# zertovitch/zip-ada

Measured on AMD Instinct MI355X. Metric: Deflate encode MB/s (Deflate_3; stream bit-exact with the CPU restatement of the reference, Ada parity unpinned), higher is better.
Workload: dtype u8

## Files before the change

### zip-ada_amd/csrc/zada_api.hip

```cpp
#include <hip/hip_runtime.h>
#include <stdint.h>
#include <stdio.h>
#include <string.h>
#include <algorithm>
#include <new>
#include <atomic>
#include <mutex>
#include <condition_variable>
#include <functional>
#include <thread>
#include "../../include/zada.h"
#include "zada_internal.h"
#include "zada_bt4.h"

struct zada_ctx { zada::Ctx c; };

namespace zada {

thread_local std::string *tls_err = nullptr;
int hip_check(Ctx *c, hipError_t e, const char *what) {
  if (e == hipSuccess) return 0;
  char buf[256];
  snprintf(buf, sizeof buf, "%s: %s", what, hipGetErrorString(e));
  if (tls_err) *tls_err = buf; else c->err = buf;
// ... 890 lines not shown
  lzma_free(&z->c);
  free_workspace(&z->c);
  for (hipEvent_t e : z->c.ev_pool) hipEventDestroy(e);
  if (z->c.stream2) hipStreamDestroy(z->c.stream2);
  if (z->c.crc_host) hipHostFree(z->c.crc_host);
  for (int b = 0; b < 2 * MAX_COPY_LANES; b++) { if (z->c.stage[b]) hipHostFree(z->c.stage[b]); if (z->c.ev_stage[b]) hipEventDestroy(z->c.ev_stage[b]); }
  for (int t = 0; t < MAX_COPY_LANES; t++) { if (z->c.stream_in[t]) hipStreamDestroy(z->c.stream_in[t]); if (z->c.ev_in[t]) hipEventDestroy(z->c.ev_in[t]); }
  if (z->c.bstage) hipHostFree(z->c.bstage);
  if (z->c.btab) hipHostFree(z->c.btab);
  if (z->c.ev_input) hipEventDestroy(z->c.ev_input);
  if (z->c.ev_out) hipEventDestroy(z->c.ev_out);
  if (z->c.ev_dlim) hipEventDestroy(z->c.ev_dlim);
  if (z->c.stream) hipStreamDestroy(z->c.stream);
  delete z;
}

zada_ctx *zada_create(int device) {
  int ndev = 0;
  if (hipGetDeviceCount(&ndev) != hipSuccess || ndev <= 0 || device < 0 || device >= ndev) return nullptr;
  if (hipSetDevice(device) != hipSuccess) return nullptr;
  zada_ctx *z = new (std::nothrow) zada_ctx();
  if (!z) return nullptr;
  z->c.device = device;
  if (hipStreamCreate(&z->c.stream) != hipSuccess ||
      hipHostMalloc((void **)&z->c.crc_host, (CRC_HOST_TOP + 64) * 4, hipHostMallocDefault) != hipSuccess ||
      hipStreamCreate(&z->c.stream2) != hipSuccess || hipEventCreateWithFlags(&z->c.ev_input, hipEventDisableTiming) != hipSuccess ||
      hipEventCreateWithFlags(&z->c.ev_out, hipEventDisableTiming) != hipSuccess || hipEventCreateWithFlags(&z->c.ev_dlim, hipEventDisableTiming) != hipSuccess) { (void)hipGetLastError(); ctx_release(z); return nullptr; }
  if (const char *e = getenv("ZADA_BUDGET")) z->c.knob_budget = atoi(e);
  if (const char *e = getenv("ZADA_INNER_BUDGET")) z->c.knob_inner_budget = atoi(e);
  if (const char *e = getenv("ZADA_LINK_RUN")) { const int v = atoi(e); if (v >= 0 && v <= 64 && !(v & (v - 1))) z->c.knob_link_run = v; }
  if (const char *e = getenv("ZADA_ATOMS_PCT")) { if (atoi(e) >= 1 && atoi(e) <= 100) z->c.knob_atoms_pct = atoi(e); }
  if (const char *e = getenv("ZADA_CD_FILTER")) z->c.knob_cd_filter = atoi(e) != 0;
  if (const char *e = getenv("ZADA_EXACT_RESPEC")) { if (atoi(e) >= 0) z->c.knob_exact_respec = atoi(e); }
  if (const char *e = getenv("ZADA_MAX_DEMAND_ROUNDS")) { if (atoi(e) > 0) z->c.knob_max_demand_rounds = atoi(e); }
  if (const char *e = getenv("ZADA_SHARD_KIB")) { if (atoi(e) >= 64 && atoi(e) % 64 == 0) z->c.knob_shard_kib = atoi(e); }
  return z;
}

void zada_destroy(zada_ctx *z) {
  if (!z) return;
  hipSetDevice(z->c.device);
  ctx_release(z);
}

const char *zada_last_error(const zada_ctx *z) { return z ? z->c.err.c_str() : "no context"; }

int zada_set_knob(zada_ctx *z, const char *name, int value) {
  if (!z || !name) return ZADA_E_INVALID;
  if (!strcmp(name, "budget")) z->c.knob_budget = value;
  else if (!strcmp(name, "inner_budget")) z->c.knob_inner_budget = value;
  else if (!strcmp(name, "link_run")) { if (value < 0 || value > 64 || (value & (value - 1))) return ZADA_E_INVALID; z->c.knob_link_run = value; }
  else if (!strcmp(name, "span_mib")) { if (value < 1 || value > 3968) return ZADA_E_INVALID; z->c.knob_span_mib = value; }
  else if (!strcmp(name, "bunzip_batch_mib")) { if (value < 16 || value > 262144) return ZADA_E_INVALID; z->c.knob_bunzip_batch_mib = value; }
  else if (!strcmp(name, "bz_batch_mib")) { if (value < 1 || value > 2048) return ZADA_E_INVALID; z->c.knob_bz_batch_mib = value; }
  else if (!strcmp(name, "bz_span_mib")) { if (value < 24 || value > 3072) return ZADA_E_INVALID; z->c.knob_bz_span_mib = value; }
  else if (!strcmp(name, "bz_batch_melems")) { if (value < 1 || value > 1536) return ZADA_E_INVALID; z->c.knob_bz_batch_melems = value; }
  else if (!strcmp(name, "bz_tail_pct")) { if (value < 0 || value > 50) return ZADA_E_INVALID; z->c.knob_bz_tail_pct = value; }
  else if (!strcmp(name, "bz_text_order")) { if (value < 0 || value > 1) return ZADA_E_INVALID; z->c.knob_bz_text_order = value; }
  else if (!strcmp(name, "bz_pipeline")) { if (value < 0 || value > 1) return ZADA_E_INVALID; z->c.knob_bz_pipeline = value; }
  else if (!strcmp(name, "bz_pipe_prio")) { if (value < 0 || value > 1) return ZADA_E_INVALID; z->c.knob_bz_pipe_prio = value; }
  else if (!strcmp(name, "bz_list_rows")) { if (value < 0 || value > 8192) return ZADA_E_INVALID; z->c.knob_bz_list_rows = value; }
  else if (!strcmp(name, "bz_split")) { if (value < 0 || value > 1) return ZADA_E_INVALID; z->c.knob_bz_split = value; }
  else if (!strcmp(name, "bz_small_wg")) { if (value < 0 || value > 1) return ZADA_E_INVALID; z->c.knob_bz_small_wg = value; }
  else if (!strcmp(name, "bz_lists")) { if (value < -1) return ZADA_E_INVALID; z->c.knob_bz_lists = value; }
  else if (!strcmp(name, "batch_mib")) { if (value < 1 || value > 1024) return ZADA_E_INVALID; z->c.knob_batch_mib = value; }
  else if (!strcmp(name, "atoms_pct")) { if (value < 1 || value > 100) return ZADA_E_INVALID; z->c.knob_atoms_pct = value; z->c.ws.cap_atoms = 0; }
  else if (!strcmp(name, "fix_stride")) { if (value < 0 || value > (int)PTOK_STRIDE) return ZADA_E_INVALID; z->c.knob_fix_stride = value; z->c.ws.cap_n = 0; }
  else if (!strcmp(name, "cd_list_cap")) { if (value < 0) return ZADA_E_INVALID; z->c.knob_cd_list_cap = value; }
  else if (!strcmp(name, "cd_filter")) { if (value < 0 || value > 1) return ZADA_E_INVALID; z->c.knob_cd_filter = value; }
  else if (!strcmp(name, "exact_respec")) { if (value < 0) return ZADA_E_INVALID; z->c.knob_exact_respec = value; }
  else if (!strcmp(name, "max_demand_rounds")) z->c.knob_max_demand_rounds = value > 0 ? value : 12;
  else if (!strcmp(name, "shard_kib")) { if (value < 64 || value % 64) return ZADA_E_INVALID; z->c.knob_shard_kib = value; }
  else if (!strcmp(name, "lzma_dict")) { if (value < 0) return ZADA_E_INVALID; z->c.knob_lzma_dict = value; }
  else if (!strcmp(name, "lzma_chunk")) { if (value < -1 || (value > 0 && value < 256)) return ZADA_E_INVALID; z->c.knob_lzma_chunk = value; }
  else if (!strcmp(name, "lzma_pool")) { if (value < 0) return ZADA_E_INVALID; z->c.knob_lzma_pool = value; }
  else if (!strcmp(name, "lzma_pool_fixed")) { if (value < 0 || value > 1) return ZADA_E_INVALID; z->c.knob_lzma_pool_fixed = value; }
  else if (!strcmp(name, "lzma_waves")) { if (value != 0 && value != 1 && value != 4) return ZADA_E_INVALID; z->c.knob_lzma_waves = value; }
  else if (!strcmp(name, "lzma_lit_mib")) { if (value < 1) return ZADA_E_INVALID; z->c.knob_lzma_lit_mib = value; }
  else if (!strcmp(name, "lzma_segment")) { if (value < -1 || (value > 0 && (value < 13 || value > 30))) return ZADA_E_INVALID; z->c.knob_lzma_segment = value; }
  else return ZADA_E_INVALID;
  return ZADA_OK;
}

constexpr int COPY_LANES = ZADA_COPY_LANES;
static_assert(COPY_LANES <= MAX_COPY_LANES, "staging buffers");
static_assert(COPY_LANES == ARR_LANES, "the arriving input's lanes use the staging buffers of copy_in's");
constexpr uint64_t COPY_MT_MIN = 64ull << 20;
static bool ensure_staging(Ctx *c, int lanes) {
  for (int b = 0; b < 2 * lanes; b++) {
    if (c->stage[b]) continue;
    if (hipHostMalloc((void **)&c->stage[b], STAGE_BYTES, hipHostMallocDefault) != hipSuccess ||
        hipEventCreateWithFlags(&c->ev_stage[b], hipEventDisableTiming) != hipSuccess) {
      if (c->stage[b]) { hipHostFree(c->stage[b]); c->stage[b] = nullptr; }
      (void)hipGetLastError();
      return false;
    }
  }
  return true;
}

static void copy_in_lane(Ctx *c, void *d_dst, const uint8_t *src, uint64_t n, int t, int T) {
  uint64_t i = 0;
  for (uint64_t o = (uint64_t)t * STAGE_BYTES; o < n; o += (uint64_t)T * STAGE_BYTES, i++) {
// ... 1164 lines not shown
```

### zip-ada_amd/csrc/zada_internal.h

```cpp
#pragma once
#ifndef ZADA_NLEVELS
#define ZADA_NLEVELS 2
#endif
#include <hip/hip_runtime.h>
#include <stdint.h>
#include <string>
#include <functional>
#include <vector>
#include "zada_logic.h"
#include "zada_sizing.h"

namespace zada {

constexpr int ZADA_E_HIP_ = -3;

#ifndef ZADA_PCHUNK
#define ZADA_PCHUNK 512
#endif
constexpr uint32_t PCHUNK = ZADA_PCHUNK;
static_assert(PCHUNK > 258, "k_fix_forward: a 258-byte step crosses at most one chunk boundary");
constexpr uint32_t PTOK_STRIDE = PCHUNK + 640;
constexpr uint32_t FIX_STRIDE_SMALL = 128;
constexpr uint32_t CRC_CHUNK = 4096, CRC_SUB = 256;
constexpr uint64_t IN_PAD = 1024;
// ... 203 lines not shown
  void *bzd = nullptr;
  void *ulz = nullptr;
  void *lz_tab = nullptr; size_t cap_lz_tab = 0;
  void *lz_save = nullptr; size_t cap_lz_save = 0;
  void *lz_lit = nullptr; size_t cap_lz_lit = 0;
  bool lz_last_lit_hbm = false;
  int knob_lzma_lit_mib = 12288;
  int lzma_launches = 0;
  std::vector<uint8_t> lz_resume;
  bool lz_stopped = false;
  bool lz_run_stopped = false;
  uint64_t lz_last_n = 0, lz_last_out_off = 0;
  void *bt4 = nullptr;
  uint32_t bt4_buckets = 0, bt4_long = 0, bt4_overflow = 0;
  uint32_t bt4_pool_grown = 0;
  int knob_lzma_pool_fixed = 0;
  uint32_t bt4_reruns = 0;
  int knob_lzma_waves = 0;
  int knob_lzma_segment = 0;
  int knob_lzma_pool = 0;
  std::vector<hipEvent_t> ev_pool;
  std::vector<std::pair<const char *, hipEvent_t>> marks;
  std::vector<std::pair<const char *, float>> timing;
  bool timing_on = true;
  uint32_t last_nblocks = 0;
  int knob_budget = -1;
  int knob_max_demand_rounds = 12;
  int knob_atoms_pct = 50;
  int knob_fix_stride = 0;
  int knob_cd_list_cap = 0;
  int knob_cd_filter = 1;
  int knob_exact_respec = 32768;
  int knob_bz_pipe_prio = 0;
  int knob_link_run = 0;
  int knob_inner_budget = 0;
  int knob_span_mib = 2048;
  int knob_batch_mib = 512;
  int knob_bunzip_batch_mib = 8192;
  int knob_bz_batch_mib = 256;
  int knob_bz_span_mib = 1024;
  int knob_bz_text_order = 1;
  int knob_bz_tail_pct = 0;
  int knob_bz_batch_melems = 768;
  int knob_bz_lists = -1;
  int knob_bz_pipeline = 1;
  int knob_bz_list_rows = 0;
  int knob_bz_split = 1;
  int knob_bz_small_wg = 1;
  int knob_lzma_dict = 0;
  int knob_lzma_chunk = 0;
  int knob_shard_kib = 1 << 20;
  void tmark(const char *name);
  void tbegin();
  void tend();
};

extern thread_local std::string *tls_err;
int hip_check(Ctx *c, hipError_t e, const char *what);
void bz2_destroy(Ctx *c);
void crypt_destroy(Ctx *c);
void inflate_destroy(Ctx *c);
int inflate_crc_entries(Ctx *c, uint32_t E, const uint64_t *out, const uint64_t *out_len, uint32_t *regs);
void bunzip2_destroy(Ctx *c);
void unlzma_destroy(Ctx *c);
void crypt_update_keys(uint32_t keys[3], uint8_t by);
uint8_t crypt_code(const uint32_t keys[3]);
// ... 76 lines not shown
```

### zip-ada_amd/csrc/zada_logic.h

```cpp
#pragma once
#include <type_traits>
#include <stdint.h>

#if defined(__HIPCC__)
#define ZADA_HD __host__ __device__ __forceinline__
#else
#define ZADA_HD inline
#endif

namespace zada {

constexpr uint32_t TOK_MATCH = 0x80000000u;
ZADA_HD uint32_t tok_match(uint32_t len, uint32_t dist) { return TOK_MATCH | (len << 16) | dist; }
ZADA_HD bool tok_is_match(uint32_t t) { return (t & TOK_MATCH) != 0; }
ZADA_HD uint32_t tok_len(uint32_t t) { return tok_is_match(t) ? ((t >> 16) & 0x1FF) : 1u; }
ZADA_HD uint32_t tok_dist(uint32_t t) { return t & 0xFFFF; }

constexpr int MIN_MATCH = 3, MAX_MATCH = 258, MAX_DIST = 32506, TOO_FAR = 4096;
constexpr int WSIZE = 32768;

struct LzConfig { int good, lazy, nice, chain; };
ZADA_HD LzConfig lz_config(int level) {
  switch (level) {
    case 4: return {4, 4, 16, 16};
// ... 69 lines not shown
  s.avail = 1;
  return 0xFFFFFFFFu;
}


struct MatchPair { uint32_t full, quarter; };
constexpr uint32_t M_GUESS = 0x80000000u, M_DEMAND = 0x40000000u, M_BYSPEC = 0x20000000u, M_HAVEQ = 0x10000000u, M_VALUE = 0x01FFFFFFu;
constexpr uint32_t M_BEAT_SHIFT = 25, M_BEAT_MAX = 127;
struct NoGuess { ZADA_HD void operator()(uint32_t, uint32_t, uint32_t, uint32_t) const {} };
struct ParseIO { const uint8_t *in; uint64_t n; const MatchPair *M; LzConfig cfg; const uint32_t *segend; };
struct Layout { const uint32_t *segend; uint64_t n; };
struct ExitState { uint32_t pos, kind; };

struct BitmapWriter {
  uint32_t *bits; uint64_t word; uint32_t acc;
  ZADA_HD void init(uint32_t *b, uint64_t first) { bits = b; acc = 0; word = first; }
  ZADA_HD void set(uint64_t p) {
    uint64_t w = p >> 5;
    while (word < w) { bits[word] = acc; acc = 0; word++; }
    acc |= 1u << (p & 31);
  }
  ZADA_HD void finish(uint64_t last) {
    while (word < last) { bits[word] = acc; acc = 0; word++; }
    bits[word] = acc;
  }
};

struct DirectFetch { const MatchPair *M; ZADA_HD MatchPair operator()(uint32_t p) const { return M[p]; } };
template <typename F> struct has_byte { template <typename U> static auto test(int) -> decltype(((U *)0)->byte(0u), char()); template <typename U> static long test(...); static const bool value = sizeof(test<F>(0)) == 1; };
template <typename F> ZADA_HD typename std::enable_if<has_byte<typename std::remove_reference<F>::type>::value, uint32_t>::type fetch_byte(F &f, const uint8_t *, uint32_t p) { return f.byte(p); }
template <typename F> ZADA_HD typename std::enable_if<!has_byte<typename std::remove_reference<F>::type>::value, uint32_t>::type fetch_byte(F &, const uint8_t *in, uint32_t p) { return in[p]; }
struct DirectSink { uint32_t *tok; uint32_t &ntok; ZADA_HD void push(uint32_t t) { tok[ntok++] = t; } };
struct CappedSink { uint32_t *tok; uint32_t &ntok; uint32_t cap; uint32_t *overflow; ZADA_HD void push(uint32_t t) { if (ntok < cap) tok[ntok] = t; else if (overflow) *overflow = 1u; ntok++; } };
template <typename Sink, typename OnTop, typename OnGuess, typename Fetch>
ZADA_HD void run_parser(ParseState &s, const ParseIO &io, Sink &&sink, OnTop &&on_top, OnGuess &&on_guess, Fetch &&fetch) {
  for (;;) {
    if ((uint64_t)s.p >= io.n) {
      if (s.avail) { sink.push(io.in[io.n - 1]); s.avail = 0; s.mlen = 2; }
      return;
    }
    if (on_top(s)) return;
    const uint64_t la = io.n - s.p;
    const bool srch = parse_searches(s, io.cfg, la);
    uint32_t m = 0;
    if (srch) {
      const MatchPair mm = fetch(s.p);
      if (mm.full & M_GUESS) on_guess(s.p, mm.full, mm.quarter, s.mlen);
      m = (parse_need_quarter(s, io.cfg) ? mm.quarter : mm.full) & M_VALUE;
    }
    const uint32_t bb = s.avail ? fetch_byte(fetch, io.in, s.p - 1) : 0;
    const uint32_t t = parse_step(s, m, srch, bb);
    if (t != 0xFFFFFFFFu) sink.push(t);
  }
}

template <typename Sink, typename OnGuess, typename Fetch>
ZADA_HD void parse_spec_chunk_to(const ParseIO &io, uint32_t k, uint32_t chunk, Sink &&sink,
                                 uint32_t *Fbits, uint32_t *Lbits, ExitState &ex, OnGuess on_guess, Fetch &&fetch) {
  const uint64_t c0 = (uint64_t)k * chunk, c1 = (c0 + chunk < io.n) ? c0 + chunk : io.n;
  ParseState s{(uint32_t)c0, 0, 2, 0};
  BitmapWriter fw, lw;
  fw.init(Fbits, c0 >> 5); lw.init(Lbits, c0 >> 5);
  ExitState e; e.pos = (uint32_t)io.n; e.kind = SYNC_F;
  run_parser(s, io, sink, [&](const ParseState &st) {
    int kind = sync_kind(st);
    if (kind == SYNC_NONE) return false;
    if ((uint64_t)st.p >= c1) { e.pos = st.p; e.kind = (uint32_t)kind; return true; }
    if (kind == SYNC_F) fw.set(st.p); else lw.set(st.p);
    return false;
  }, on_guess, fetch);
  const uint64_t lastw = c1 > c0 ? (c1 - 1) >> 5 : c0 >> 5;
  fw.finish(lastw);
  lw.finish(lastw);
  ex = e;
}
template <typename OnGuess, typename Fetch>
ZADA_HD void parse_spec_chunk(const ParseIO &io, uint32_t k, uint32_t chunk, uint32_t *tok, uint32_t &ntok,
                              uint32_t *Fbits, uint32_t *Lbits, ExitState &ex, OnGuess on_guess, Fetch &&fetch) {
  parse_spec_chunk_to(io, k, chunk, DirectSink{tok, ntok}, Fbits, Lbits, ex, on_guess, fetch);
}
ZADA_HD void parse_spec_chunk(const ParseIO &io, uint32_t k, uint32_t chunk, uint32_t *tok, uint32_t &ntok,
                              uint32_t *Fbits, uint32_t *Lbits, ExitState &ex) {
  parse_spec_chunk_to(io, k, chunk, DirectSink{tok, ntok}, Fbits, Lbits, ex, NoGuess(), DirectFetch{io.M});
}

template <typename OnGuess, typename Fetch>
ZADA_HD void parse_fix_chunk(const ParseIO &io, uint32_t k, uint32_t chunk, ExitState entry,
                             const uint32_t *spec_tok, uint32_t spec_cnt, const uint32_t *Fbits, const uint32_t *Lbits,
                             ExitState spec_exit, uint32_t *tok, uint32_t &ntok, uint32_t &take, uint32_t &u0, ExitState &new_exit,
                             OnGuess on_guess, Fetch &&fetch, uint32_t tok_cap = 0xFFFFFFFFu, uint32_t *tok_overflow = nullptr) {
  const uint64_t c0 = (uint64_t)k * chunk, c1 = (c0 + chunk < io.n) ? c0 + chunk : io.n;
  u0 = entry.kind == SYNC_L ? entry.pos - 1 : entry.pos;
  ntok = 0;
  if ((uint64_t)entry.pos >= c1) {
    new_exit = entry; take = spec_cnt;
    return;
  }
  ParseState s{entry.pos, entry.kind == SYNC_L ? 1u : 0u, 2, 0};
  bool synced = false;
  ExitState e; e.pos = (uint32_t)io.n; e.kind = SYNC_F;
  run_parser(s, io, CappedSink{tok, ntok, tok_cap, tok_overflow}, [&](const ParseState &st) {
    int kind = sync_kind(st);
    if (kind == SYNC_NONE) return false;
    if ((uint64_t)st.p >= c1) { e.pos = st.p; e.kind = (uint32_t)kind; return true; }
    uint32_t wbits = (kind == SYNC_F ? Fbits : Lbits)[st.p >> 5];
    if ((wbits >> (st.p & 31)) & 1) { synced = true; e.pos = st.p; e.kind = (uint32_t)kind; return true; }
    return false;
  }, on_guess, fetch);
  if (synced) {
    const uint32_t u = e.kind == SYNC_L ? e.pos - 1 : e.pos;
    uint32_t cur = (uint32_t)c0, j = 0;
    while (cur < u) { cur += tok_len(spec_tok[j]); j++; }
    take = j;
    new_exit = spec_exit;
  } else {
    take = spec_cnt;
    new_exit = e;
  }
}
ZADA_HD void parse_fix_chunk(const ParseIO &io, uint32_t k, uint32_t chunk, ExitState entry,
                                    const uint32_t *spec_tok, uint32_t spec_cnt, const uint32_t *Fbits, const uint32_t *Lbits,
                                    ExitState spec_exit, uint32_t *tok, uint32_t &ntok, uint32_t &take, uint32_t &u0, ExitState &new_exit) {
  parse_fix_chunk(io, k, chunk, entry, spec_tok, spec_cnt, Fbits, Lbits, spec_exit, tok, ntok, take, u0, new_exit, NoGuess(), DirectFetch{io.M});
}

template <typename T>
ZADA_HD void patch_dist_stats(T *sd) {
  int used = 0;
  for (int i = 0; i < 32; i++) if (sd[i] != 0) used++;
  if (used == 0) { sd[0] = 1; sd[1] = 1; }
  else if (used == 1) { if (sd[0] == 0) sd[0] = 1; else sd[1] = 1; }
}

ZADA_HD void tweak_for_better_rle(uint32_t *counts, int counts_len, uint8_t *good) {
  int length = counts_len, stride;
  uint32_t symbol, sum, limit, new_count;
  for (int i = 0; i < counts_len; i++) good[i] = 0;
  for (;;) { if (length == 0) return; if (counts[length - 1] != 0) break; length--; }
  symbol = counts[0]; stride = 0;
  for (int i = 0; i <= length; i++) {
    if (i == length || counts[i] != symbol) {
      if ((symbol == 0 && stride >= 5) || (symbol != 0 && stride >= 7))
        for (int k = 0; k < stride; k++) good[i - k - 1] = 1;
      stride = 1;
      if (i != length) symbol = counts[i];
    } else stride++;
  }
  stride = 0; limit = counts[0]; sum = 0;
  for (int i = 0; i <= length; i++) {
    bool brk = (i == length) || good[i] || (i > 0 && good[i - 1]);
    if (!brk) { int64_t d = (int64_t)counts[i] - (int64_t)limit; if (d < 0) d = -d; brk = d >= 4; }
// ... 79 lines not shown
```

### zip-ada_amd/csrc/zada_lz.hip

```cpp
#include <hip/hip_runtime.h>
#include <mutex>
#include <stdint.h>
#include "zada_logic.h"
#include "zada_internal.h"
#include <chrono>
#include <stdio.h>
#include <stdlib.h>
#include <vector>

namespace zada {

typedef uint32_t __attribute__((aligned(1))) u32u;
typedef uint64_t __attribute__((aligned(1))) u64u;
#define RL(v, j) ((uint32_t)__builtin_amdgcn_readlane((int)(v), (j)))
#define RL64(v, j) ((uint64_t)RL((uint32_t)(v), (j)) | ((uint64_t)RL((uint32_t)((v) >> 32), (j)) << 32))

#ifndef ZADA_NO_XCD_MAP
__device__ __forceinline__ uint32_t xcd_block() {
  const uint32_t n = gridDim.x, full = n & ~7u, b = blockIdx.x;
  return b < full ? (b & 7u) * (full >> 3) + (b >> 3) : b;
}
#else
__device__ __forceinline__ uint32_t xcd_block() { return blockIdx.x; }
#endif
// ... 1692 lines not shown
struct WaveSink {
  uint32_t *dst; uint32_t n;
  __device__ void push(uint32_t t) { if ((threadIdx.x & 63) == 0) dst[n] = t; n++; }
};
constexpr int PX_WAVES = 4;
__global__ void __launch_bounds__(64 * PX_WAVES) k_parse_spec_exact(ParseIO io, uint32_t nchunks, uint32_t *__restrict__ spec_tok, uint32_t *__restrict__ spec_cnt,
                                                                     uint32_t *__restrict__ Fbits, uint32_t *__restrict__ Lbits, ExitState *__restrict__ exits,
                                                                     WaveExact wx, const uint32_t *__restrict__ list, const uint32_t *__restrict__ list_n, uint32_t exact_max) {
  __shared__ uint64_t recs[PX_WAVES][PX_RECS];
  const int lane = threadIdx.x & 63, w = threadIdx.x >> 6;
  const uint32_t nl = *list_n, stride = gridDim.x * PX_WAVES;
  if (nl > exact_max) return;
  for (uint32_t i = blockIdx.x * PX_WAVES + w; i < nl; i += stride) {
    const uint32_t k = list[i];
    if (k >= nchunks) continue;
    ParseIO cio = io;
    if (io.segend) cio.n = io.segend[((uint64_t)k * PCHUNK) >> 15] & 0x7FFFFFFFu;
    const uint32_t c0 = k * PCHUNK;
    {
      const uint64_t *src = (const uint64_t *)(io.M + c0);
      const uint32_t have = (uint64_t)c0 + PX_RECS <= io.n ? PX_RECS : (uint32_t)(io.n - c0);
      for (uint32_t j = lane; j < have; j += 64) recs[w][j] = src[j];
    }
    __builtin_amdgcn_wave_barrier();
    WaveFetch wf; wf.recs = recs[w]; wf.c0 = c0; wf.Mg = io.M; wf.wx = &wx;
    WaveSink ts; ts.dst = spec_tok + (uint64_t)k * PTOK_STRIDE; ts.n = 0;
    ExitState ex;
    parse_spec_chunk_to(cio, k, PCHUNK, ts, Fbits, Lbits, ex, NoGuess(), wf);
    if (lane == 0) { spec_cnt[k] = ts.n; exits[k] = ex; }
    __builtin_amdgcn_wave_barrier();
  }
}

__global__ void k_parse_fix(ParseIO io, uint32_t nchunks, const uint32_t *__restrict__ spec_tok, const uint32_t *__restrict__ spec_cnt,
                            const uint32_t *__restrict__ Fbits, const uint32_t *__restrict__ Lbits,
                            const ExitState *__restrict__ spec_exits, ExitState *__restrict__ true_exits,
                            uint32_t *__restrict__ fix_tok, uint32_t *__restrict__ fix_cnt,
                            uint32_t *__restrict__ take_from, uint32_t *__restrict__ start_pos,
                            const uint8_t *__restrict__ dirty_in, uint8_t *__restrict__ dirty_out,
                            uint32_t *__restrict__ n_changed, DemandMarker dm, ExitState entry0, uint32_t fix_stride, uint32_t *__restrict__ fix_overflow) {
  uint32_t k = blockIdx.x * blockDim.x + threadIdx.x;
  if (k >= nchunks) return;
  if (!dirty_in[k]) return;
  ExitState entry = entry0;
  if (k > 0) entry = true_exits[k - 1];
  if (io.segend) {
    const uint32_t se = io.segend[((uint64_t)k * PCHUNK) >> 15];
    io.n = se & 0x7FFFFFFFu;
    if ((se >> 31) && ((k * PCHUNK) & 32767u) == 0) entry = ExitState{k * PCHUNK, SYNC_F};
  }
  const ExitState old_exit = true_exits[k];
  ExitState new_exit;
  uint32_t ntok = 0, take = 0, u0 = 0;
  parse_fix_chunk(io, k, PCHUNK, entry, spec_tok + (uint64_t)k * PTOK_STRIDE, spec_cnt[k], Fbits, Lbits, spec_exits[k],
                  fix_tok + (uint64_t)k * fix_stride, ntok, take, u0, new_exit, dm, DirectFetch{io.M}, fix_stride, fix_overflow);
  fix_cnt[k] = ntok;
  take_from[k] = take;
  start_pos[k] = u0;
  true_exits[k] = new_exit;
  if (k + 1 < nchunks && (new_exit.pos != old_exit.pos || new_exit.kind != old_exit.kind)) {
    dirty_out[k + 1] = 1;
    atomicAdd(n_changed, 1u);
    atomicMin(n_changed + 1, k);
  }
}

__global__ void __launch_bounds__(64) k_fix_forward(ParseIO io, uint32_t nchunks, ExitState *__restrict__ true_exits,
                                                    uint8_t *__restrict__ dirty_out, uint32_t *__restrict__ n_changed) {
  const uint32_t k = n_changed[1];
  if (k >= nchunks || 258 < io.cfg.lazy || io.segend) return;
  const ExitState e0 = true_exits[k];
  if (e0.kind != SYNC_F) return;
  const int lane = threadIdx.x;
  for (uint64_t q0 = e0.pos;; q0 += 258ull * 64) {
    const uint64_t q = q0 + 258ull * lane;
    bool good = false;
    if (q + 258 <= io.n) { const uint32_t f = io.M[q].full; good = !(f & M_GUESS) && ((f & M_VALUE) >> 16) == 258u; }
    const unsigned long long bad = ~__ballot(good);
    const int nvalid = bad ? __ffsll((long long)bad) - 1 : 64;
    if (lane <= nvalid && (lane > 0 || q0 != e0.pos)) {
      const uint64_t c1 = (q / PCHUNK) * PCHUNK;
      if (q - c1 < 258 && c1 >= PCHUNK) {
        const uint32_t kk = (uint32_t)(c1 / PCHUNK) - 1;
        if (kk > k && kk < nchunks) {
          const ExitState old = true_exits[kk];
          if (old.pos != (uint32_t)q || old.kind != SYNC_F) {
// ... 243 lines not shown
#endif
    c->tmark("prev_links");
    if (!job.need) {
      if (nseg > 1) {
        cross_links(1, nseg);
        cross_dist();
      }
      hipLaunchKernelGGL(k_bucket_limits, dim3(nseg), dim3(256), 0, st, L, cfg.chain, cfg.chain >> 2, W.S3, W.bsc3, W.dlim, W.dlim_bits, W.segmax, W.heavy, 0u);
    }
  }
#ifdef ZADA_CD_STATS
  { unsigned long long h[16]; hipDeviceSynchronize(); hipMemcpyFromSymbol(h, HIP_SYMBOL(g_cd_dbg), sizeof h);
    fprintf(stderr, "[k_cross_dist level-4 walks] %llu walks (%.1f %% of the positions), %llu steps (%.2f per walk), found %llu (%.1f %%), no step %llu, > 8 steps %llu, > 64 steps %llu, steps of the walks that found nothing %llu, gave-up restarts %llu\n",
            h[0], 100.0 * h[0] / n, h[1], (double)h[1] / (h[0] ? h[0] : 1), h[2], 100.0 * h[2] / (h[0] ? h[0] : 1), h[3], h[4], h[5], h[6], h[7]);
    fprintf(stderr, "[k_cross_dist level-4 walks] > 32 steps %llu, > 128 %llu, > 256 %llu, > 512 %llu, > 1024 %llu, longest %llu\n", h[8], h[9], h[10], h[11], h[12], h[13]);
    for (int q = 0; q < 16; q++) h[q] = 0; hipMemcpyToSymbol(HIP_SYMBOL(g_cd_dbg), h, sizeof h); }
#endif
  c->tmark("cross_links");
  const uint32_t nbm = (uint32_t)((n + MB - 1) / MB);
  const uint32_t nch = (uint32_t)((n + PCHUNK - 1) / PCHUNK);
  const int max_rounds = c->knob_max_demand_rounds;
  int budget_env = c->knob_budget >= 0 ? c->knob_budget : (n < (2u << 20) ? 0 : n < (512u << 20) ? 8 : 6);
  if (budget_env < 1) budget_env = 1 << 20;
  const uint32_t nbd = (uint32_t)((n + DMB - 1) / DMB);
  hipMemsetAsync(W.blk_demand, 0, (size_t)nbd * 4, st);
  hipMemsetAsync(W.dbits, 0, (size_t)nbd * (DMB / 8), st);
  hipMemsetAsync(W.n_demand, 0, 4, st);
  hipLaunchKernelGGL(k_match, dim3(nbm), dim3(1024), MATCH_LDS, st, W.in, L, W.lprev[NLEVELS - 1], dpl, W.M, cfg.nice,
                     budget_env, (unsigned long long *)W.dbg, W.lprev[0], budget_env > c->knob_inner_budget ? c->knob_inner_budget : 0);
  c->tmark("match");
  ParseIO io; io.in = W.in; io.n = n; io.M = W.M; io.cfg = cfg; io.segend = job.segend;
  DemandMarker dm; dm.M = W.M; dm.blk_demand = W.blk_demand; dm.n_demand = W.n_demand; dm.by = M_BYSPEC; dm.dbits = W.dbits;
  DemandMarker dmf = dm; dmf.by = 0;
  int rounds = 0, demand_rounds = 0;
  bool valve_used = false;
  static const bool round_stats = getenv("ZADA_ROUND_STATS") != nullptr;
  const ExitState entry0 = job.entry_known ? job.entry : ExitState{0, SYNC_F};
  const uint32_t kE = job.entry_known ? (entry0.pos / PCHUNK < nch ? entry0.pos / PCHUNK : nch) : 0u;
  hipMemsetAsync(W.n_changed + 6, 0, 4, st);
  bool restart = false, first_again = false;
  for (bool first = true;; first = false) {
    if (first_again) { first = true; first_again = false; }
    const bool beat_valid = !first;
    if (first) hipLaunchKernelGGL(k_parse_spec, dim3((nch + 63) / 64), dim3(64), 0, st, io, nch,
                                  W.spec_tok, W.spec_cnt, W.Fbits, W.Lbits, W.spec_exits, dm, (const uint32_t *)nullptr, (const uint32_t *)nullptr, 0u);
    else {
      hipMemsetAsync(W.n_changed + 2, 0, 4, st);
      hipLaunchKernelGGL(k_list_flagged, dim3((nch + 1023) / 1024), dim3(1024), 0, st, W.chg, nch, W.offsets, W.n_changed + 2);
      const uint32_t exact_max = c->knob_exact_respec > 0 ? (uint32_t)c->knob_exact_respec : 0u;
      if (exact_max) {
        WaveExact wx; wx.in = W.in; wx.L = L; wx.dp = dpl; wx.rp = rpt; wx.tailsK = W.ltails[NLEVELS - 1]; wx.M = W.M; wx.nice_cfg = cfg.nice; wx.resume = W.lprev[0];
        hipLaunchKernelGGL(k_parse_spec_exact, dim3(256 * 5), dim3(64 * PX_WAVES), 0, st, io, nch, W.spec_tok, W.spec_cnt, W.Fbits, W.Lbits, W.spec_exits,
                           wx, (const uint32_t *)W.offsets, (const uint32_t *)(W.n_changed + 2), exact_max);
      }
      DemandMarker dmt = dm; dmt.track = true;
      hipLaunchKernelGGL(k_parse_spec, dim3((nch + 63) / 64), dim3(64), 0, st, io, nch,
                         W.spec_tok, W.spec_cnt, W.Fbits, W.Lbits, W.spec_exits, dmt, (const uint32_t *)W.offsets, (const uint32_t *)(W.n_changed + 2), exact_max);
    }
    hipMemcpyAsync(W.true_exits, W.spec_exits, (size_t)nch * sizeof(ExitState), hipMemcpyDeviceToDevice, st);
    if (kE > 0) hipLaunchKernelGGL(k_seed_entry, dim3((kE + 255) / 256), dim3(256), 0, st, W.true_exits, kE, entry0);
    hipMemsetAsync(W.dirty[0], 1, nch, st);
    int cur = 0, it = 0;
    uint32_t ndem = 0;
    bool slow = false;
    for (;;) {
      hipMemsetAsync(W.dirty[cur ^ 1], 0, nch, st);
      hipMemsetAsync(W.n_changed, 0, 4, st);
      hipMemsetAsync(W.n_changed + 1, 0xFF, 4, st);
      hipLaunchKernelGGL(k_parse_fix, dim3((nch + 63) / 64), dim3(64), 0, st, io, nch,
                         W.spec_tok, W.spec_cnt, W.Fbits, W.Lbits, W.spec_exits, W.true_exits, W.fix_tok, W.fix_cnt,
                         W.take_from, W.start_pos, W.dirty[cur], W.dirty[cur ^ 1], W.n_changed, dmf, entry0, W.fix_stride, W.n_changed + 6);
      hipLaunchKernelGGL(k_fix_forward, dim3(1), dim3(64), 0, st, io, nch, W.true_exits, W.dirty[cur ^ 1], W.n_changed);
      uint32_t changed = 0, fix_ovf = 0;
      hipMemcpyAsync(&changed, W.n_changed, 4, hipMemcpyDeviceToHost, st);
      hipMemcpyAsync(&ndem, W.n_demand, 4, hipMemcpyDeviceToHost, st);
      if (W.fix_stride < PTOK_STRIDE) hipMemcpyAsync(&fix_ovf, W.n_changed + 6, 4, hipMemcpyDeviceToHost, st);
      if (hip_check(c, hipStreamSynchronize(st), "parse_fix")) return ZADA_E_HIP_;
      rounds++;
      if (fix_ovf) {
        uint32_t *bigger = nullptr;
        const uint64_t nch_cap = W.cap_n / PCHUNK + 2;
        if (hipMalloc(&bigger, nch_cap * (uint64_t)PTOK_STRIDE * 4) != hipSuccess) { (void)hipGetLastError(); c->err = "out of device memory (splice tokens)"; return -2; }
        W.allocs.push_back(bigger);
        W.fix_tok = bigger; W.fix_stride = PTOK_STRIDE;
        c->fix_grown++;
        hipMemsetAsync(W.n_changed + 6, 0, 4, st);
        restart = true;
        break;
      }
      if (changed == 0) break;
      if (++it >= 32 && !valve_used) { slow = true; break; }
      cur ^= 1;
    }
    if (round_stats) {
      uint32_t nl = 0, nmark = 0;
      if (!first) hipMemcpy(&nl, W.n_changed + 2, 4, hipMemcpyDeviceToHost);
      { std::vector<uint32_t> hb(nbd); hipMemcpy(hb.data(), W.blk_demand, (size_t)nbd * 4, hipMemcpyDeviceToHost); for (uint32_t v : hb) nmark += v != 0; }
      fprintf(stderr, "[lz round %d] %s parse of %u chunks, splice iterations so far %d, blocks with demanded positions %u of %u, demand %u%s\n", demand_rounds, first || nl > (uint32_t)(c->knob_exact_respec > 0 ? c->knob_exact_respec : 0) ? "speculative" : "exact",
              first ? nch : nl, rounds, nmark, nbd, ndem, slow ? " (slow splice)" : "");
    }
#ifdef ZADA_RESPEC_STATS
    if (!first) { unsigned long long h[4]; hipDeviceSynchronize(); hipMemcpyFromSymbol(h, HIP_SYMBOL(g_respec_dbg), sizeof h); fprintf(stderr, "[respec round %d] %llu chunks parsed again, %llu of them with the same tokens and exit as before\n", demand_rounds, h[0], h[1]); h[0] = h[1] = 0; hipMemcpyToSymbol(HIP_SYMBOL(g_respec_dbg), h, sizeof h); }
#endif
    if (restart) { restart = false; first_again = true; continue; }
    if (ndem == 0 && !slow) break;
    demand_rounds++;
    if (demand_rounds > 1000) { c->err = "demand loop did not converge"; return ZADA_E_HIP_; }
    hipMemsetAsync(W.n_demand, 0, 4, st);
    hipMemsetAsync(W.chg, 0, nch, st);
    if ((demand_rounds == max_rounds || slow) && !valve_used) {
      valve_used = true;
      hipLaunchKernelGGL(k_demand_all, dim3((uint32_t)((n + 255) / 256)), dim3(256), 0, st, L, W.M, W.blk_demand, W.dbits);
    }
    hipLaunchKernelGGL(k_match_demand, dim3(nbd), dim3(DM_THREADS), DM_LDS, st, W.in, L, dpl, rpt, W.ltails[NLEVELS - 1], W.M, cfg.nice,
                       W.blk_demand, W.dbits, W.chg, W.spec_exits, W.lprev[0], beat_valid);
    hipMemsetAsync(W.blk_demand, 0, (size_t)nbd * 4, st);
#ifdef ZADA_DM_STATS
    { unsigned long long h[8]; hipDeviceSynchronize(); hipMemcpyFromSymbol(h, HIP_SYMBOL(g_dm_dbg), sizeof h);
      fprintf(stderr, "[k_match_demand round %d] %llu blocks, %.1f marked positions and %.1f scans per block; cycles per block: staging %.0f, list %.0f, phase A %.0f, phase B %.0f\n", demand_rounds, h[4],
              (double)h[5] / (h[4] ? h[4] : 1), (double)h[6] / (h[4] ? h[4] : 1), (double)h[0] / (h[4] ? h[4] : 1), (double)h[1] / (h[4] ? h[4] : 1), (double)h[2] / (h[4] ? h[4] : 1), (double)h[3] / (h[4] ? h[4] : 1));
      for (int q = 0; q < 8; q++) h[q] = 0; hipMemcpyToSymbol(HIP_SYMBOL(g_dm_dbg), h, sizeof h); }
#endif
  }
  c->demand_rounds += demand_rounds;
  c->parse_rounds += rounds;
  c->tmark("parse");
  const uint32_t k0 = job.tok_lo / PCHUNK, k1 = job.final ? nch : job.tok_hi / PCHUNK, nk = k1 - k0;
  if (nk == 0) { c->err = "empty shard"; return -1; }
  hipLaunchKernelGGL(k_tok_count, dim3((nch + 255) / 256), dim3(256), 0, st, nch, W.spec_cnt, W.fix_cnt, W.take_from, W.counts);
  exclusive_scan_u32(st, W.counts + k0, W.offsets, W.scan_sums, W.n_changed, nk);
  struct { uint32_t total; ExitState ex, warm; } h;
// ... 19 lines not shown
```

Before: 9493.

## Resolve guessed matches inline with wave-cooperative exact search in respec and splice parse

Splits the parser loop into fetch and step halves so that GPU kernels can, between them, run a wave-cooperative exact match search for lanes whose match lookup is only a guess. A new lane-per-chunk respeculation kernel and a templated splice-fix kernel use this inline settle instead of recording demand for later match-demand rounds. The goal is fewer demand rounds and fewer round trips to the host after the first pass. In exchange, every lane in a wave waits on the serialized per-lane exact searches, and the inline kernels are limited to 64-thread blocks.

```diff
diff --git a/zip-ada_amd/csrc/zada_api.hip b/zip-ada_amd/csrc/zada_api.hip
--- a/zip-ada_amd/csrc/zada_api.hip
+++ b/zip-ada_amd/csrc/zada_api.hip
@@ -946,6 +946,7 @@
   if (const char *e = getenv("ZADA_ATOMS_PCT")) { if (atoi(e) >= 1 && atoi(e) <= 100) z->c.knob_atoms_pct = atoi(e); }
   if (const char *e = getenv("ZADA_CD_FILTER")) z->c.knob_cd_filter = atoi(e) != 0;
   if (const char *e = getenv("ZADA_EXACT_RESPEC")) { if (atoi(e) >= 0) z->c.knob_exact_respec = atoi(e); }
+  if (const char *e = getenv("ZADA_INLINE_EXACT")) { if (atoi(e) == 0 || atoi(e) == 1) z->c.knob_inline_exact = atoi(e); }
   if (const char *e = getenv("ZADA_MAX_DEMAND_ROUNDS")) { if (atoi(e) > 0) z->c.knob_max_demand_rounds = atoi(e); }
   if (const char *e = getenv("ZADA_SHARD_KIB")) { if (atoi(e) >= 64 && atoi(e) % 64 == 0) z->c.knob_shard_kib = atoi(e); }
   return z;
@@ -983,6 +984,7 @@
   else if (!strcmp(name, "cd_list_cap")) { if (value < 0) return ZADA_E_INVALID; z->c.knob_cd_list_cap = value; }
   else if (!strcmp(name, "cd_filter")) { if (value < 0 || value > 1) return ZADA_E_INVALID; z->c.knob_cd_filter = value; }
   else if (!strcmp(name, "exact_respec")) { if (value < 0) return ZADA_E_INVALID; z->c.knob_exact_respec = value; }
+  else if (!strcmp(name, "inline_exact")) { if (value < 0 || value > 1) return ZADA_E_INVALID; z->c.knob_inline_exact = value; }
   else if (!strcmp(name, "max_demand_rounds")) z->c.knob_max_demand_rounds = value > 0 ? value : 12;
   else if (!strcmp(name, "shard_kib")) { if (value < 64 || value % 64) return ZADA_E_INVALID; z->c.knob_shard_kib = value; }
   else if (!strcmp(name, "lzma_dict")) { if (value < 0) return ZADA_E_INVALID; z->c.knob_lzma_dict = value; }
diff --git a/zip-ada_amd/csrc/zada_internal.h b/zip-ada_amd/csrc/zada_internal.h
--- a/zip-ada_amd/csrc/zada_internal.h
+++ b/zip-ada_amd/csrc/zada_internal.h
@@ -259,6 +259,7 @@
   int knob_cd_filter = 1;
   int knob_exact_respec = 32768;
   int knob_bz_pipe_prio = 0;
+  int knob_inline_exact = 1;
   int knob_link_run = 0;
   int knob_inner_budget = 0;
   int knob_span_mib = 2048;
diff --git a/zip-ada_amd/csrc/zada_logic.h b/zip-ada_amd/csrc/zada_logic.h
--- a/zip-ada_amd/csrc/zada_logic.h
+++ b/zip-ada_amd/csrc/zada_logic.h
@@ -125,47 +125,69 @@
 template <typename F> ZADA_HD typename std::enable_if<!has_byte<typename std::remove_reference<F>::type>::value, uint32_t>::type fetch_byte(F &, const uint8_t *in, uint32_t p) { return in[p]; }
 struct DirectSink { uint32_t *tok; uint32_t &ntok; ZADA_HD void push(uint32_t t) { tok[ntok++] = t; } };
 struct CappedSink { uint32_t *tok; uint32_t &ntok; uint32_t cap; uint32_t *overflow; ZADA_HD void push(uint32_t t) { if (ntok < cap) tok[ntok] = t; else if (overflow) *overflow = 1u; ntok++; } };
+template <typename Sink, typename OnTop, typename Fetch>
+ZADA_HD bool parse_turn_fetch(ParseState &s, const ParseIO &io, Sink &&sink, OnTop &&on_top, Fetch &&fetch, bool &srch, MatchPair &mm) {
+  if ((uint64_t)s.p >= io.n) {
+    if (s.avail) { sink.push(io.in[io.n - 1]); s.avail = 0; s.mlen = 2; }
+    return false;
+  }
+  if (on_top(s)) return false;
+  const uint64_t la = io.n - s.p;
+  srch = parse_searches(s, io.cfg, la);
+  if (srch) mm = fetch(s.p);
+  return true;
+}
+template <typename Sink, typename OnGuess, typename Fetch>
+ZADA_HD void parse_turn_step(ParseState &s, const ParseIO &io, Sink &&sink, OnGuess &&on_guess, Fetch &&fetch, bool srch, const MatchPair &mm) {
+  uint32_t m = 0;
+  if (srch) {
+    if (mm.full & M_GUESS) on_guess(s.p, mm.full, mm.quarter, s.mlen);
+    m = (parse_need_quarter(s, io.cfg) ? mm.quarter : mm.full) & M_VALUE;
+  }
+  const uint32_t bb = s.avail ? fetch_byte(fetch, io.in, s.p - 1) : 0;
+  const uint32_t t = parse_step(s, m, srch, bb);
+  if (t != 0xFFFFFFFFu) sink.push(t);
+}
 template <typename Sink, typename OnTop, typename OnGuess, typename Fetch>
 ZADA_HD void run_parser(ParseState &s, const ParseIO &io, Sink &&sink, OnTop &&on_top, OnGuess &&on_guess, Fetch &&fetch) {
   for (;;) {
-    if ((uint64_t)s.p >= io.n) {
-      if (s.avail) { sink.push(io.in[io.n - 1]); s.avail = 0; s.mlen = 2; }
-      return;
-    }
-    if (on_top(s)) return;
-    const uint64_t la = io.n - s.p;
-    const bool srch = parse_searches(s, io.cfg, la);
-    uint32_t m = 0;
-    if (srch) {
-      const MatchPair mm = fetch(s.p);
-      if (mm.full & M_GUESS) on_guess(s.p, mm.full, mm.quarter, s.mlen);
-      m = (parse_need_quarter(s, io.cfg) ? mm.quarter : mm.full) & M_VALUE;
-    }
-    const uint32_t bb = s.avail ? fetch_byte(fetch, io.in, s.p - 1) : 0;
-    const uint32_t t = parse_step(s, m, srch, bb);
-    if (t != 0xFFFFFFFFu) sink.push(t);
-  }
-}
-
-template <typename Sink, typename OnGuess, typename Fetch>
-ZADA_HD void parse_spec_chunk_to(const ParseIO &io, uint32_t k, uint32_t chunk, Sink &&sink,
-                                 uint32_t *Fbits, uint32_t *Lbits, ExitState &ex, OnGuess on_guess, Fetch &&fetch) {
-  const uint64_t c0 = (uint64_t)k * chunk, c1 = (c0 + chunk < io.n) ? c0 + chunk : io.n;
-  ParseState s{(uint32_t)c0, 0, 2, 0};
-  BitmapWriter fw, lw;
-  fw.init(Fbits, c0 >> 5); lw.init(Lbits, c0 >> 5);
-  ExitState e; e.pos = (uint32_t)io.n; e.kind = SYNC_F;
-  run_parser(s, io, sink, [&](const ParseState &st) {
+    bool srch = false;
+    MatchPair mm{0, 0};
+    if (!parse_turn_fetch(s, io, sink, on_top, fetch, srch, mm)) return;
+    parse_turn_step(s, io, sink, on_guess, fetch, srch, mm);
+  }
+}
+
+struct SpecChunk {
+  uint64_t c0, c1; BitmapWriter fw, lw; ExitState e;
+  ZADA_HD void begin(const ParseIO &io, uint32_t k, uint32_t chunk, uint32_t *Fbits, uint32_t *Lbits, ParseState &s) {
+    c0 = (uint64_t)k * chunk; c1 = (c0 + chunk < io.n) ? c0 + chunk : io.n;
+    s = ParseState{(uint32_t)c0, 0, 2, 0};
+    fw.init(Fbits, c0 >> 5); lw.init(Lbits, c0 >> 5);
+    e.pos = (uint32_t)io.n; e.kind = SYNC_F;
+  }
+  ZADA_HD bool operator()(const ParseState &st) {
     int kind = sync_kind(st);
     if (kind == SYNC_NONE) return false;
     if ((uint64_t)st.p >= c1) { e.pos = st.p; e.kind = (uint32_t)kind; return true; }
     if (kind == SYNC_F) fw.set(st.p); else lw.set(st.p);
     return false;
-  }, on_guess, fetch);
-  const uint64_t lastw = c1 > c0 ? (c1 - 1) >> 5 : c0 >> 5;
-  fw.finish(lastw);
-  lw.finish(lastw);
-  ex = e;
+  }
+  ZADA_HD void end(ExitState &ex) {
+    const uint64_t lastw = c1 > c0 ? (c1 - 1) >> 5 : c0 >> 5;
+    fw.finish(lastw);
+    lw.finish(lastw);
+    ex = e;
+  }
+};
+template <typename Sink, typename OnGuess, typename Fetch>
+ZADA_HD void parse_spec_chunk_to(const ParseIO &io, uint32_t k, uint32_t chunk, Sink &&sink,
+                                 uint32_t *Fbits, uint32_t *Lbits, ExitState &ex, OnGuess on_guess, Fetch &&fetch) {
+  ParseState s;
+  SpecChunk top;
+  top.begin(io, k, chunk, Fbits, Lbits, s);
+  run_parser(s, io, sink, top, on_guess, fetch);
+  top.end(ex);
 }
 template <typename OnGuess, typename Fetch>
 ZADA_HD void parse_spec_chunk(const ParseIO &io, uint32_t k, uint32_t chunk, uint32_t *tok, uint32_t &ntok,
@@ -177,39 +199,54 @@
   parse_spec_chunk_to(io, k, chunk, DirectSink{tok, ntok}, Fbits, Lbits, ex, NoGuess(), DirectFetch{io.M});
 }
 
-template <typename OnGuess, typename Fetch>
-ZADA_HD void parse_fix_chunk(const ParseIO &io, uint32_t k, uint32_t chunk, ExitState entry,
-                             const uint32_t *spec_tok, uint32_t spec_cnt, const uint32_t *Fbits, const uint32_t *Lbits,
-                             ExitState spec_exit, uint32_t *tok, uint32_t &ntok, uint32_t &take, uint32_t &u0, ExitState &new_exit,
-                             OnGuess on_guess, Fetch &&fetch, uint32_t tok_cap = 0xFFFFFFFFu, uint32_t *tok_overflow = nullptr) {
-  const uint64_t c0 = (uint64_t)k * chunk, c1 = (c0 + chunk < io.n) ? c0 + chunk : io.n;
-  u0 = entry.kind == SYNC_L ? entry.pos - 1 : entry.pos;
-  ntok = 0;
-  if ((uint64_t)entry.pos >= c1) {
-    new_exit = entry; take = spec_cnt;
-    return;
-  }
-  ParseState s{entry.pos, entry.kind == SYNC_L ? 1u : 0u, 2, 0};
-  bool synced = false;
-  ExitState e; e.pos = (uint32_t)io.n; e.kind = SYNC_F;
-  run_parser(s, io, CappedSink{tok, ntok, tok_cap, tok_overflow}, [&](const ParseState &st) {
+struct FixChunk {
+  uint64_t c0, c1; const uint32_t *Fbits, *Lbits; bool synced; ExitState e;
+  ZADA_HD bool begin(const ParseIO &io, uint32_t k, uint32_t chunk, ExitState entry, uint32_t spec_cnt, const uint32_t *Fb, const uint32_t *Lb,
+                     ParseState &s, uint32_t &ntok, uint32_t &take, uint32_t &u0, ExitState &new_exit) {
+    c0 = (uint64_t)k * chunk; c1 = (c0 + chunk < io.n) ? c0 + chunk : io.n;
+    Fbits = Fb; Lbits = Lb;
+    u0 = entry.kind == SYNC_L ? entry.pos - 1 : entry.pos;
+    ntok = 0;
+    if ((uint64_t)entry.pos >= c1) {
+      new_exit = entry; take = spec_cnt;
+      return false;
+    }
+    s = ParseState{entry.pos, entry.kind == SYNC_L ? 1u : 0u, 2, 0};
+    synced = false;
+    e.pos = (uint32_t)io.n; e.kind = SYNC_F;
+    return true;
+  }
+  ZADA_HD bool operator()(const ParseState &st) {
     int kind = sync_kind(st);
     if (kind == SYNC_NONE) return false;
     if ((uint64_t)st.p >= c1) { e.pos = st.p; e.kind = (uint32_t)kind; return true; }
     uint32_t wbits = (kind == SYNC_F ? Fbits : Lbits)[st.p >> 5];
     if ((wbits >> (st.p & 31)) & 1) { synced = true; e.pos = st.p; e.kind = (uint32_t)kind; return true; }
     return false;
-  }, on_guess, fetch);
-  if (synced) {
-    const uint32_t u = e.kind == SYNC_L ? e.pos - 1 : e.pos;
-    uint32_t cur = (uint32_t)c0, j = 0;
-    while (cur < u) { cur += tok_len(spec_tok[j]); j++; }
-    take = j;
-    new_exit = spec_exit;
-  } else {
-    take = spec_cnt;
-    new_exit = e;
-  }
+  }
+  ZADA_HD void end(const uint32_t *spec_tok, uint32_t spec_cnt, ExitState spec_exit, uint32_t &take, ExitState &new_exit) {
+    if (synced) {
+      const uint32_t u = e.kind == SYNC_L ? e.pos - 1 : e.pos;
+      uint32_t cur = (uint32_t)c0, j = 0;
+      while (cur < u) { cur += tok_len(spec_tok[j]); j++; }
+      take = j;
+      new_exit = spec_exit;
+    } else {
+      take = spec_cnt;
+      new_exit = e;
+    }
+  }
+};
+template <typename OnGuess, typename Fetch>
+ZADA_HD void parse_fix_chunk(const ParseIO &io, uint32_t k, uint32_t chunk, ExitState entry,
+                             const uint32_t *spec_tok, uint32_t spec_cnt, const uint32_t *Fbits, const uint32_t *Lbits,
+                             ExitState spec_exit, uint32_t *tok, uint32_t &ntok, uint32_t &take, uint32_t &u0, ExitState &new_exit,
+                             OnGuess on_guess, Fetch &&fetch, uint32_t tok_cap = 0xFFFFFFFFu, uint32_t *tok_overflow = nullptr) {
+  ParseState s;
+  FixChunk top;
+  if (!top.begin(io, k, chunk, entry, spec_cnt, Fbits, Lbits, s, ntok, take, u0, new_exit)) return;
+  run_parser(s, io, CappedSink{tok, ntok, tok_cap, tok_overflow}, top, on_guess, fetch);
+  top.end(spec_tok, spec_cnt, spec_exit, take, new_exit);
 }
 ZADA_HD void parse_fix_chunk(const ParseIO &io, uint32_t k, uint32_t chunk, ExitState entry,
                                     const uint32_t *spec_tok, uint32_t spec_cnt, const uint32_t *Fbits, const uint32_t *Lbits,
diff --git a/zip-ada_amd/csrc/zada_lz.hip b/zip-ada_amd/csrc/zada_lz.hip
--- a/zip-ada_amd/csrc/zada_lz.hip
+++ b/zip-ada_amd/csrc/zada_lz.hip
@@ -1748,26 +1748,91 @@
   }
 }
 
-__global__ void k_parse_fix(ParseIO io, uint32_t nchunks, const uint32_t *__restrict__ spec_tok, const uint32_t *__restrict__ spec_cnt,
+__device__ __forceinline__ void wave_settle(const WaveExact &wx, bool g, uint32_t p, MatchPair &mm) {
+  const int lane = threadIdx.x & 63;
+  for (unsigned long long b = __ballot(g); b; b &= b - 1) {
+    const int j = __ffsll((long long)b) - 1;
+    MatchPair og; og.full = RL(mm.full, j); og.quarter = RL(mm.quarter, j);
+    const MatchPair r = wx.search((uint64_t)RL(p, j), og);
+    if (lane == j) mm = r;
+  }
+}
+__global__ void __launch_bounds__(64) k_parse_spec_inline(ParseIO io, uint32_t nchunks, uint32_t *__restrict__ spec_tok, uint32_t *__restrict__ spec_cnt,
+                                                          uint32_t *__restrict__ Fbits, uint32_t *__restrict__ Lbits, ExitState *__restrict__ exits,
+                                                          WaveExact wx, const uint32_t *__restrict__ list, const uint32_t *__restrict__ list_n, uint32_t exact_max) {
+  uint32_t k = blockIdx.x * 64 + threadIdx.x;
+  const uint32_t nl = *list_n;
+  if (nl <= exact_max || blockIdx.x * 64 >= nl) return;
+  bool mine = k < nl;
+  if (mine) { k = list[k]; mine = k < nchunks; }
+  if (!mine) k = 0;
+  if (mine && io.segend) io.n = io.segend[((uint64_t)k * PCHUNK) >> 15] & 0x7FFFFFFFu;
+  __shared__ uint64_t lines[8 * 64];
+  __shared__ uint32_t tbuf[PS_TOKS * 64];
+  __shared__ uint32_t blines[PS_BWORDS * 64];
+  LineFetch lf; lf.M = io.M; lf.slot = lines + threadIdx.x; lf.tag = 0xFFFFFFFFu; lf.in = io.in; lf.bslot = blines + threadIdx.x; lf.btag = 0xFFFFFFFFu;
+  TokSink ts; ts.dst = spec_tok + (uint64_t)k * PTOK_STRIDE; ts.buf = tbuf + threadIdx.x; ts.n = 0;
+  ParseState s{0, 0, 2, 0};
+  SpecChunk top;
+  if (mine) top.begin(io, k, PCHUNK, Fbits, Lbits, s);
+  bool done = !mine;
+  do {
+    bool srch = false;
+    MatchPair mm{0, 0};
+    if (!done) done = !parse_turn_fetch(s, io, ts, top, lf, srch, mm);
+    wave_settle(wx, !done && srch && (mm.full & M_GUESS), s.p, mm);
+    if (!done) parse_turn_step(s, io, ts, NoGuess(), lf, srch, mm);
+  } while (__any(!done));
+  if (!mine) return;
+  ExitState ex;
+  top.end(ex);
+  ts.flush();
+  spec_cnt[k] = ts.n;
+  exits[k] = ex;
+}
+
+template <bool INLINE_EXACT>
+__global__ void __launch_bounds__(INLINE_EXACT ? 64 : 1024) k_parse_fix(ParseIO io, uint32_t nchunks, const uint32_t *__restrict__ spec_tok, const uint32_t *__restrict__ spec_cnt,
                             const uint32_t *__restrict__ Fbits, const uint32_t *__restrict__ Lbits,
                             const ExitState *__restrict__ spec_exits, ExitState *__restrict__ true_exits,
                             uint32_t *__restrict__ fix_tok, uint32_t *__restrict__ fix_cnt,
                             uint32_t *__restrict__ take_from, uint32_t *__restrict__ start_pos,
                             const uint8_t *__restrict__ dirty_in, uint8_t *__restrict__ dirty_out,
-                            uint32_t *__restrict__ n_changed, DemandMarker dm, ExitState entry0, uint32_t fix_stride, uint32_t *__restrict__ fix_overflow) {
+                            uint32_t *__restrict__ n_changed, DemandMarker dm, ExitState entry0, uint32_t fix_stride, uint32_t *__restrict__ fix_overflow, WaveExact wx) {
   uint32_t k = blockIdx.x * blockDim.x + threadIdx.x;
-  if (k >= nchunks) return;
-  if (!dirty_in[k]) return;
+  const bool mine = k < nchunks && dirty_in[k];
+  if (INLINE_EXACT) {
+    if (!__any(mine)) return;
+    if (!mine) k = 0;
+  } else if (!mine) return;
   ExitState entry = entry0;
-  if (k > 0) entry = true_exits[k - 1];
-  if (io.segend) {
+  if (mine && k > 0) entry = true_exits[k - 1];
+  if (mine && io.segend) {
     const uint32_t se = io.segend[((uint64_t)k * PCHUNK) >> 15];
     io.n = se & 0x7FFFFFFFu;
     if ((se >> 31) && ((k * PCHUNK) & 32767u) == 0) entry = ExitState{k * PCHUNK, SYNC_F};
   }
-  const ExitState old_exit = true_exits[k];
+  ExitState old_exit{0, 0};
+  if (mine) old_exit = true_exits[k];
   ExitState new_exit;
   uint32_t ntok = 0, take = 0, u0 = 0;
+  if (INLINE_EXACT) {
+    ParseState s{0, 0, 2, 0};
+    FixChunk top;
+    const bool runs = mine && top.begin(io, k, PCHUNK, entry, spec_cnt[k], Fbits, Lbits, s, ntok, take, u0, new_exit);
+    CappedSink sink{fix_tok + (uint64_t)k * fix_stride, ntok, fix_stride, fix_overflow};
+    DirectFetch df{io.M};
+    bool done = !runs;
+    do {
+      bool srch = false;
+      MatchPair mm{0, 0};
+      if (!done) done = !parse_turn_fetch(s, io, sink, top, df, srch, mm);
+      wave_settle(wx, !done && srch && (mm.full & M_GUESS), s.p, mm);
+      if (!done) parse_turn_step(s, io, sink, NoGuess(), df, srch, mm);
+    } while (__any(!done));
+    if (!mine) return;
+    if (runs) top.end(spec_tok + (uint64_t)k * PTOK_STRIDE, spec_cnt[k], spec_exits[k], take, new_exit);
+  } else
   parse_fix_chunk(io, k, PCHUNK, entry, spec_tok + (uint64_t)k * PTOK_STRIDE, spec_cnt[k], Fbits, Lbits, spec_exits[k],
                   fix_tok + (uint64_t)k * fix_stride, ntok, take, u0, new_exit, dm, DirectFetch{io.M}, fix_stride, fix_overflow);
   fix_cnt[k] = ntok;
@@ -2077,6 +2142,8 @@
   ParseIO io; io.in = W.in; io.n = n; io.M = W.M; io.cfg = cfg; io.segend = job.segend;
   DemandMarker dm; dm.M = W.M; dm.blk_demand = W.blk_demand; dm.n_demand = W.n_demand; dm.by = M_BYSPEC; dm.dbits = W.dbits;
   DemandMarker dmf = dm; dmf.by = 0;
+  WaveExact wx; wx.in = W.in; wx.L = L; wx.dp = dpl; wx.rp = rpt; wx.tailsK = W.ltails[NLEVELS - 1]; wx.M = W.M; wx.nice_cfg = cfg.nice; wx.resume = W.lprev[0];
+  const bool inline_exact = c->knob_inline_exact != 0;
   int rounds = 0, demand_rounds = 0;
   bool valve_used = false;
   static const bool round_stats = getenv("ZADA_ROUND_STATS") != nullptr;
@@ -2093,14 +2160,15 @@
       hipMemsetAsync(W.n_changed + 2, 0, 4, st);
       hipLaunchKernelGGL(k_list_flagged, dim3((nch + 1023) / 1024), dim3(1024), 0, st, W.chg, nch, W.offsets, W.n_changed + 2);
       const uint32_t exact_max = c->knob_exact_respec > 0 ? (uint32_t)c->knob_exact_respec : 0u;
-      if (exact_max) {
-        WaveExact wx; wx.in = W.in; wx.L = L; wx.dp = dpl; wx.rp = rpt; wx.tailsK = W.ltails[NLEVELS - 1]; wx.M = W.M; wx.nice_cfg = cfg.nice; wx.resume = W.lprev[0];
-        hipLaunchKernelGGL(k_parse_spec_exact, dim3(256 * 5), dim3(64 * PX_WAVES), 0, st, io, nch, W.spec_tok, W.spec_cnt, W.Fbits, W.Lbits, W.spec_exits,
-                           wx, (const uint32_t *)W.offsets, (const uint32_t *)(W.n_changed + 2), exact_max);
-      }
-      DemandMarker dmt = dm; dmt.track = true;
-      hipLaunchKernelGGL(k_parse_spec, dim3((nch + 63) / 64), dim3(64), 0, st, io, nch,
-                         W.spec_tok, W.spec_cnt, W.Fbits, W.Lbits, W.spec_exits, dmt, (const uint32_t *)W.offsets, (const uint32_t *)(W.n_changed + 2), exact_max);
+      if (exact_max) hipLaunchKernelGGL(k_parse_spec_exact, dim3(256 * 5), dim3(64 * PX_WAVES), 0, st, io, nch, W.spec_tok, W.spec_cnt, W.Fbits, W.Lbits, W.spec_exits,
+                                        wx, (const uint32_t *)W.offsets, (const uint32_t *)(W.n_changed + 2), exact_max);
+      if (inline_exact) hipLaunchKernelGGL(k_parse_spec_inline, dim3((nch + 63) / 64), dim3(64), 0, st, io, nch, W.spec_tok, W.spec_cnt, W.Fbits, W.Lbits, W.spec_exits,
+                                           wx, (const uint32_t *)W.offsets, (const uint32_t *)(W.n_changed + 2), exact_max);
+      else {
+        DemandMarker dmt = dm; dmt.track = true;
+        hipLaunchKernelGGL(k_parse_spec, dim3((nch + 63) / 64), dim3(64), 0, st, io, nch,
+                           W.spec_tok, W.spec_cnt, W.Fbits, W.Lbits, W.spec_exits, dmt, (const uint32_t *)W.offsets, (const uint32_t *)(W.n_changed + 2), exact_max);
+      }
     }
     hipMemcpyAsync(W.true_exits, W.spec_exits, (size_t)nch * sizeof(ExitState), hipMemcpyDeviceToDevice, st);
     if (kE > 0) hipLaunchKernelGGL(k_seed_entry, dim3((kE + 255) / 256), dim3(256), 0, st, W.true_exits, kE, entry0);
@@ -2112,9 +2180,9 @@
       hipMemsetAsync(W.dirty[cur ^ 1], 0, nch, st);
       hipMemsetAsync(W.n_changed, 0, 4, st);
       hipMemsetAsync(W.n_changed + 1, 0xFF, 4, st);
-      hipLaunchKernelGGL(k_parse_fix, dim3((nch + 63) / 64), dim3(64), 0, st, io, nch,
+      hipLaunchKernelGGL(!first && inline_exact ? k_parse_fix<true> : k_parse_fix<false>, dim3((nch + 63) / 64), dim3(64), 0, st, io, nch,
                          W.spec_tok, W.spec_cnt, W.Fbits, W.Lbits, W.spec_exits, W.true_exits, W.fix_tok, W.fix_cnt,
-                         W.take_from, W.start_pos, W.dirty[cur], W.dirty[cur ^ 1], W.n_changed, dmf, entry0, W.fix_stride, W.n_changed + 6);
+                         W.take_from, W.start_pos, W.dirty[cur], W.dirty[cur ^ 1], W.n_changed, dmf, entry0, W.fix_stride, W.n_changed + 6, wx);
       hipLaunchKernelGGL(k_fix_forward, dim3(1), dim3(64), 0, st, io, nch, W.true_exits, W.dirty[cur ^ 1], W.n_changed);
       uint32_t changed = 0, fix_ovf = 0;
       hipMemcpyAsync(&changed, W.n_changed, 4, hipMemcpyDeviceToHost, st);
@@ -2141,7 +2209,7 @@
       uint32_t nl = 0, nmark = 0;
       if (!first) hipMemcpy(&nl, W.n_changed + 2, 4, hipMemcpyDeviceToHost);
       { std::vector<uint32_t> hb(nbd); hipMemcpy(hb.data(), W.blk_demand, (size_t)nbd * 4, hipMemcpyDeviceToHost); for (uint32_t v : hb) nmark += v != 0; }
-      fprintf(stderr, "[lz round %d] %s parse of %u chunks, splice iterations so far %d, blocks with demanded positions %u of %u, demand %u%s\n", demand_rounds, first || nl > (uint32_t)(c->knob_exact_respec > 0 ? c->knob_exact_respec : 0) ? "speculative" : "exact",
+      fprintf(stderr, "[lz round %d] %s parse of %u chunks, splice iterations so far %d, blocks with demanded positions %u of %u, demand %u%s\n", demand_rounds, first ? "speculative" : nl > (uint32_t)(c->knob_exact_respec > 0 ? c->knob_exact_respec : 0) ? (inline_exact ? "lane-per-chunk exact" : "speculative") : "exact",
               first ? nch : nl, rounds, nmark, nbd, ndem, slow ? " (slow splice)" : "");
     }
 #ifdef ZADA_RESPEC_STATS
```

After: 9537, median of 6. Within noise of the previous version (+0.5%).
